# cmu-ci-lab/MitsubaER

Measured on AMD Instinct MI355X. Metric: Mpaths/sec (curved-ray heterogeneous volume); roofline = measured HBM GB/s of the dominant kernel vs peak, higher is better.
Workload: dtype f32; 1 GPU; configs[2]: 256^3 sigma_t grid + 256^3 linear-gradient RIF, RK4 eikonal curved rays, HG g=0.8, 512^2 x 256 spp; grid=256, spp_job=256, spp_per_gpu=256, pipelines_per_gpu=4, stepper=rk4, rif_interp=trilinear, layout=brick27, estimator=volpath + delta tracking on eikonal rays, ratio-tracking NEE, device=AMD Radeon Graphics, cus=256

## Files before the change

### mitsubaer_amd/csrc/mer_api.hip

```cpp
#include "mer_internal.hpp"
#define MER_USE_DEVICE(ctx) do { if (ctx) (void) hipSetDevice((ctx)->device); } while (0)
#include "mer_kernels.hpp"
#include <algorithm>
#include <functional>
#include <utility>

using namespace mer;

namespace { thread_local std::string g_create_error; }

namespace mer {

using FetchKinds = std::integer_sequence<int, RIFK_ACOUSTIC, MER_RIF_TRILINEAR, RIFK_DENSE_BUF, RIFK_CELL8, RIFK_CELL8_BUF, RIFK_BRICK27_BUF, RIFK_BRICK27, MER_RIF_BSPLINE3>;
using Steppers = std::integer_sequence<int, MER_STEP_VERLET, MER_STEP_RK4>;
template <int... Ks, typename F> static bool match_constant(std::integer_sequence<int, Ks...>, int value, F &&f) {
    return ((value == Ks && f(std::integral_constant<int, Ks>())) || ...);
}

template <typename F> static int dispatch_modes(mer_context *ctx, const mer_scene_desc *sc, F &&f) {
    const bool curved = sc->rif_mode != MER_RIF_CONST;
    const bool grid = sc->sigma_mode == MER_SIGMA_GRID;
    if (!curved) {
        if (grid) return f(std::integral_constant<bool, false>(), std::integral_constant<int, MER_RIF_TRILINEAR>(),
                           std::integral_constant<int, MER_STEP_VERLET>(), std::integral_constant<int, MER_SIGMA_GRID>(), std::integral_constant<int, 0>());
// ... 17 lines not shown

int mer_abi_version(void) { return MER_ABI_VERSION; }

int mer_context_create(int32_t device_id, mer_context **out) {
    if (!out) return 1;
    *out = nullptr;
    int ndev = 0;
    hipError_t e = hipGetDeviceCount(&ndev);
    if (e != hipSuccess || ndev <= 0) {
        g_create_error = "mer_context_create: no HIP device available (libmer has no CPU path)";
        return 1;
    }
    if (device_id < 0 || device_id >= ndev) { g_create_error = "mer_context_create: device id out of range"; return 1; }
    mer_context *ctx = new mer_context();
    ctx->device = device_id;
    if (hipSetDevice(device_id) != hipSuccess || hipGetDeviceProperties(&ctx->prop, device_id) != hipSuccess) {
        g_create_error = "mer_context_create: hipSetDevice failed"; delete ctx; return 1;
    }
    const size_t counter_bytes = sizeof(unsigned long long) * (MER_C_COUNT * MER_COUNTER_REPLICAS + 8);
    bool ok = !ctx->counters.alloc(ctx, counter_bytes) && hipMemset(ctx->counters.p, 0, counter_bytes) == hipSuccess &&
              hipEventCreate(&ctx->ev0) == hipSuccess && hipEventCreate(&ctx->ev1) == hipSuccess;
#ifdef MER_BOUNDS_CHECK
    ok = ok && !ctx->chk_buf.alloc(ctx, 4 * sizeof(unsigned long long)) && hipMemset(ctx->chk_buf.p, 0, 4 * sizeof(unsigned long long)) == hipSuccess;
    ctx->chk = ctx->chk_buf.as<unsigned long long>();
#endif
    if (!ok) { g_create_error = "mer_context_create: device allocation failed"; mer_context_destroy(ctx); return 1; }
    if (const char *e = getenv("MER_OPTIONS")) {
        std::string all(e); size_t pos = 0;
        while (pos < all.size()) {
            size_t end = all.find(',', pos); if (end == std::string::npos) end = all.size();
            const std::string kv = all.substr(pos, end - pos); const size_t eq = kv.find('=');
            if (eq != std::string::npos && mer_context_set_option(ctx, kv.substr(0, eq).c_str(), atoll(kv.c_str() + eq + 1)) != 0) {
                g_create_error = "mer_context_create: MER_OPTIONS: " + ctx->error; mer_context_destroy(ctx); return 1;
            }
            pos = end + 1;
        }
    }
    *out = ctx;
    return 0;
}

struct OptionEntry { const char *name; int64_t *p; int64_t min, max; };
static OptionEntry option_slot(mer_context *ctx, const char *name) {
    Options &o = ctx->opt;
    const int64_t ANY = INT64_MAX;
    const OptionEntry table[] = {
        {"pipes", &o.pipes, 1, MER_MAX_PIPES}, {"nslots", &o.nslots, 0, (int64_t) 1 << 28}, {"ksteps", &o.ksteps, 1, 1 << 20}, {"mq_sort", &o.mq_sort, -1, 1},
        {"connect_launches", &o.connect_launches, 1, 64}, {"adaptive_k", &o.adaptive_k, 0, 2}, {"pass_events", &o.pass_events, -ANY - 1, ANY},
        {"buffer_loads", &o.buffer_loads, -ANY - 1, ANY}, {"gen_all", &o.gen_all, -ANY - 1, ANY}, {"prefilter", &o.prefilter, 0, 5},
        {"verbose", &o.verbose, -ANY - 1, ANY}, {"debug_pixel", &o.debug_pixel, -1, ((int64_t) 1 << 31) - 1}, {"lds_bricks", &o.lds_bricks, -ANY - 1, ANY},
        {"march_lds_kb", &o.march_lds_kb, 0, 64},
        {"tile_deal", &o.tile_deal, 0, 1}, {"small_render_slots", &o.small_render_slots, 0, 1}, {"inline_walks", &o.inline_walks, 0, 1},
        {"spawn_walks", &o.spawn_walks, 0, 1}, {"grid_fit", &o.grid_fit, 0, 1}, {"check_every", &o.check_every, 1, 64},
        {"march_sort", &o.march_sort, 0, 4}, {"march_sort_major", &o.march_sort_major, 0, 1}};
    for (const auto &t : table) if (std::strcmp(t.name, name) == 0) return t;
    ctx->error = std::string("unknown option '") + name + "'";
    return OptionEntry{name, nullptr, 0, 0};
}
int mer_context_set_option(mer_context *ctx, const char *name, int64_t value) {
    MER_USE_DEVICE(ctx);
    if (!ctx || !name) return 1;
    const OptionEntry t = option_slot(ctx, name);
    if (!t.p) return 1;
    const bool nslots_too_few = t.p == &ctx->opt.nslots && value > 0 && value < MER_BLOCK * MER_MAX_PIPES;
    if (value < t.min || value > t.max || nslots_too_few) return fail(ctx, std::string("option '") + name + "': value out of range");
    *t.p = value;
    return 0;
}
int mer_context_get_option(mer_context *ctx, const char *name, int64_t *value) {
    MER_USE_DEVICE(ctx);
    if (!ctx || !name || !value) return 1;
    const OptionEntry t = option_slot(ctx, name);
    if (!t.p) return 1;
    *value = *t.p;
    return 0;
}
int mer_debug_bounds(mer_context *ctx, int32_t *enabled, uint64_t out[4]) {
    MER_USE_DEVICE(ctx);
    if (!ctx || !enabled || !out) return 1;
    out[0] = out[1] = out[2] = out[3] = 0;
    *enabled = ctx->chk != nullptr;
    if (ctx->chk) {
        HIP_CHECK(ctx, hipDeviceSynchronize());
        HIP_CHECK(ctx, hipMemcpy(out, ctx->chk, 4 * sizeof(uint64_t), hipMemcpyDeviceToHost));
        HIP_CHECK(ctx, hipMemset(ctx->chk, 0, 4 * sizeof(uint64_t)));
    }
    return 0;
}

void mer_context_destroy(mer_context *ctx) {
    if (!ctx) return;
    (void) hipSetDevice(ctx->device);
    for (Pipe &pp : ctx->pipes) {
        for (hipEvent_t e : pp.readback) if (e) (void) hipEventDestroy(e);
        if (pp.finished) (void) hipEventDestroy(pp.finished);
        for (hipEvent_t e : pp.pass_events) (void) hipEventDestroy(e);
        if (pp.own_stream) (void) hipStreamDestroy(pp.own_stream);
    }
    if (ctx->ev0) (void) hipEventDestroy(ctx->ev0);
    if (ctx->ev1) (void) hipEventDestroy(ctx->ev1);
    delete ctx;
}

const char *mer_last_error(mer_context *ctx) { return ctx ? ctx->error.c_str() : g_create_error.c_str(); }

int mer_context_set_stream(mer_context *ctx, void *hip_stream) { ctx->stream = (hipStream_t) hip_stream; return 0; }

// ... 719 lines not shown
```

### mitsubaer_amd/csrc/mer_device.hpp

```cpp
#pragma once
#include <hip/hip_runtime.h>
#include <stdint.h>
#include <stddef.h>
#include "../../include/mer.h"

#define MER_EPSILON 1e-4f
#define MER_PI 3.14159265358979323846f
#define MER_INV_FOURPI 0.07957747154594766788f
#define MER_INV_PI 0.31830988618379067154f
#define MER_INF __builtin_huge_valf()

namespace mer {

struct f3 {
    float x, y, z;
    __host__ __device__ __forceinline__ f3() {}
    __host__ __device__ __forceinline__ f3(float a, float b, float c) : x(a), y(b), z(c) {}
};
__device__ __forceinline__ f3 operator+(f3 a, f3 b) { return f3(a.x + b.x, a.y + b.y, a.z + b.z); }
__device__ __forceinline__ f3 operator-(f3 a, f3 b) { return f3(a.x - b.x, a.y - b.y, a.z - b.z); }
__device__ __forceinline__ f3 operator-(f3 a) { return f3(-a.x, -a.y, -a.z); }
__device__ __forceinline__ f3 operator*(f3 a, float s) { return f3(a.x * s, a.y * s, a.z * s); }
__device__ __forceinline__ f3 operator*(float s, f3 a) { return f3(s * a.x, s * a.y, s * a.z); }
__device__ __forceinline__ f3 operator*(f3 a, f3 b) { return f3(a.x * b.x, a.y * b.y, a.z * b.z); }
// ... 572 lines not shown
    float pad[2];
};
static_assert(sizeof(DPoint) == 32 && sizeof(DRect) == 160 && sizeof(DSpot) == 32 && sizeof(DEnvMap) == 144, "emitter records: 16-byte multiples");
struct EmitterTable { DPoint points[MER_MAX_EMITTERS]; DRect rects[MER_MAX_EMITTERS]; DSpot spots[MER_MAX_EMITTERS]; DEnvMap env; };
static_assert(offsetof(EmitterTable, spots) == offsetof(EmitterTable, rects) + sizeof(DRect) * MER_MAX_EMITTERS, "spot_table: the cones follow the rectangle table");
static_assert(offsetof(EmitterTable, env) == offsetof(EmitterTable, spots) + sizeof(DSpot) * MER_MAX_EMITTERS, "envmap_rec: the envmap record follows the cones");
static_assert(sizeof(EmitterTable) == offsetof(EmitterTable, env) + sizeof(DEnvMap), "emitter table: no padding (the host compares it bytewise)");

struct Params {
    mer_scene_desc sc;
    DGrid density, albedo, rif;
    f3    sigA, sigS, sigT;
    float medium_sampling_weight, sampling_density;
    MaxExp maxexp;
    float inv_max_density;
    float het_step;
    float aspect, cot_half_fov, par_dir[3], lens_radius, lens_focus, sensor_pad[1];
    float inv_res_x, inv_res_y;
    const float *ftable;
    float fradius, fscale;
    uint64_t seed;
    int32_t spp_begin, spp_count, spp_stride, tile_rank, tile_count;
    int32_t tiles_x, tiles_y, ntiles_mine;
    int32_t tile_skew;
    uint64_t total_work;
    float *film;
    int32_t frames, film_ch;
    float mod_phase;
    int32_t has_envmap;
    float *path_out;
    unsigned long long *counters;
    unsigned long long *work_counter;
    int32_t dbg_pixel;
    int32_t has_spot;
    uint32_t *slots; uint32_t nslots; int32_t ksteps;
    uint32_t nslots_all;
    int32_t spawn;
    uint32_t *live;
    SegQueue eq, mq[2], sq[2];
    DGrid sdf; float sdf_eps;
    SegQueue cq[2];
    uint32_t *cstate;
    unsigned long long *hitq; unsigned long long hitq_cap;
    unsigned long long *hitq_ctr;
    int32_t gen_iters, gen_all;
    uint32_t cq_row;
    int32_t mq_sort;
    int32_t msort, msort_major; float msort_o[3], msort_s[3];
    uint32_t *msorted, *msort_hist, *msort_cursor, *msort_count;
    unsigned long long *chk;
    uint64_t n_film, n_path_out;
    int32_t n_point, n_rect; const DPoint *points; const DRect *rects;
    uint8_t *side_state;
};
#define MER_LIVE_SLOTS 4096
#define MER_COUNTER_REPLICAS 64

__device__ __forceinline__ bool inside_shape(const mer_scene_desc &s, f3 p) {
    if (s.boundary == MER_BOUNDARY_SPHERE) {
        const f3 q(p.x - s.sph_center[0], p.y - s.sph_center[1], p.z - s.sph_center[2]);
        return dot(q, q) < s.sph_radius * s.sph_radius;
    }
    return p.x >= s.bmin[0] && p.x <= s.bmax[0] && p.y >= s.bmin[1] && p.y <= s.bmax[1] && p.z >= s.bmin[2] && p.z <= s.bmax[2];
}

__device__ __forceinline__ float intersect_shape(const mer_scene_desc &s, f3 o, f3 d, float mint, float maxt) {
    float nearT, farT;
    if (s.boundary == MER_BOUNDARY_SPHERE) {
        const double ox = (double) o.x - s.sph_center[0], oy = (double) o.y - s.sph_center[1], oz = (double) o.z - s.sph_center[2];
        const double dx = d.x, dy = d.y, dz = d.z;
        const double A = dx * dx + dy * dy + dz * dz, B = 2 * (dx * ox + dy * oy + dz * oz),
                     C = ox * ox + oy * oy + oz * oz - (double) s.sph_radius * s.sph_radius;
        const double disc = B * B - 4 * A * C;
        if (disc < 0) return -1.0f;
        const double root = sqrt(disc);
        const double q = B < 0 ? -0.5 * (B - root) : -0.5 * (B + root);
        double t0 = q / A, t1 = C / q;
        if (t0 > t1) { double tmp = t0; t0 = t1; t1 = tmp; }
        nearT = (float) t0; farT = (float) t1;
    } else {
        if (!aabb_intersect(s.bmin, s.bmax, o, d, nearT, farT)) return -1.0f;
    }
    if (!(nearT <= maxt && farT >= mint)) return -1.0f;
    if (nearT >= mint) return nearT;
    if (farT <= maxt) return farT;
    return -1.0f;
}

__device__ __forceinline__ void sample_ray(const Params &P, float px, float py, f3 &o, f3 &d, float &mint, float &maxt) {
    const float *cam = P.sc.cam_to_world;
    const float sx = px * P.inv_res_x, sy = py * P.inv_res_y;
    const f3 nearP((1.0f - 2.0f * sx) * P.sc.near_clip / P.cot_half_fov,
                   (1.0f - 2.0f * sy) / P.aspect * P.sc.near_clip / P.cot_half_fov, P.sc.near_clip);
    const f3 dl = normalize(nearP);
    const float invZ = 1.0f / dl.z;
    mint = P.sc.near_clip * invZ; maxt = P.sc.far_clip * invZ;
    o = f3(cam[3], cam[7], cam[11]);
    d = f3(cam[0] * dl.x + cam[1] * dl.y + cam[2] * dl.z,
           cam[4] * dl.x + cam[5] * dl.y + cam[6] * dl.z,
           cam[8] * dl.x + cam[9] * dl.y + cam[10] * dl.z);
}

__device__ __forceinline__ void square_to_disk_concentric(float u1, float u2, float &x, float &y) {
    const float r1 = 2.0f * u1 - 1.0f, r2 = 2.0f * u2 - 1.0f;
    float phi, r;
    if (r1 == 0 && r2 == 0) { r = phi = 0; }
// ... 513 lines not shown
```

### mitsubaer_amd/csrc/mer_internal.hpp

```cpp
#pragma once
#include "mer_device.hpp"
#include <cstdio>
#include <cstdlib>
#include <cstring>
#include <cmath>
#include <string>
#include <vector>
#include <map>
#include <limits>

struct mer_context;

namespace mer {

struct DeviceBuffer {
    void *p = nullptr; size_t bytes = 0;
    DeviceBuffer() = default;
    DeviceBuffer(DeviceBuffer &&o) noexcept : p(o.p), bytes(o.bytes) { o.p = nullptr; o.bytes = 0; }
    DeviceBuffer &operator=(DeviceBuffer &&o) noexcept { if (this != &o) { reset(); p = o.p; bytes = o.bytes; o.p = nullptr; o.bytes = 0; } return *this; }
    ~DeviceBuffer() { reset(); }
    void reset() { if (p) (void) hipFree(p); p = nullptr; bytes = 0; }
    void *release() { void *q = p; p = nullptr; bytes = 0; return q; }
    static int free_raw(mer_context *ctx, void *raw);
    int alloc(mer_context *ctx, size_t n);
// ... 33 lines not shown
    int32_t family = REC_FLUENCE, kind = REC_COLLISION;
    mer_fluence_desc box{};
    mer_detector_desc det{};
    int32_t frames = 0;
    DeviceBuffer dev;
    uint64_t n_keys = 0;
    int32_t n_totals = 0;
    bool timed() const { return kind == REC_TIMED; }
    bool track() const { return kind == REC_TRACK; }
    uint64_t n_cells() const { return (uint64_t) box.res[0] * (uint64_t) box.res[1] * (uint64_t) box.res[2]; }
    int32_t faces() const { return det.boundary == MER_BOUNDARY_SPHERE ? 1 : 6; }
    double *sums() const { return dev.as<double>(); }
    double *totals() const { return sums() + n_keys * 3; }
    size_t bytes() const { return (n_keys * 3 + (uint64_t) n_totals) * sizeof(double); }
};

#define MER_MAX_PIPES 4
struct Pipe {
    hipStream_t stream = nullptr, own_stream = nullptr;
    DeviceBuffer slots; uint32_t nslots = 0; DeviceBuffer live; PinnedBuffer host_live;
    enum { NQ = 7, EQ = 0, MQ = 1, SQ = 3, CQ = 5 };
    SegQueue q[NQ]{};
    DeviceBuffer q_items[NQ], q_counts[NQ], q_keys[NQ];
    DeviceBuffer cstate;
    DeviceBuffer hitq, hitq_ctr; unsigned long long hitq_cap = 0;
    hipEvent_t readback[2] = {nullptr, nullptr}, finished = nullptr;
    std::vector<hipEvent_t> pass_events;
    DeviceBuffer side_state;
    DeviceBuffer msort;
};

struct Options {
    int64_t pipes = 4;
    int64_t nslots = 0;
    int64_t ksteps = 128;
    int64_t mq_sort = -1;
    int64_t connect_launches = 2;
    int64_t adaptive_k = 0;
    int64_t pass_events = 1;
    int64_t buffer_loads = 1;
    int64_t gen_all = 0;
    int64_t prefilter = 0;
    int64_t verbose = 0;
    int64_t debug_pixel = -1;
    int64_t march_lds_kb = 0;
    int64_t tile_deal = 1;
    int64_t inline_walks = 1;
    int64_t spawn_walks = 1;
    int64_t small_render_slots = 1;
    int64_t check_every = 4;
    int64_t grid_fit = 1;
    int64_t march_sort = 0;
    int64_t march_sort_major = 0;
    int64_t lds_bricks = 0;
};

}

struct mer_context {
    int device = 0;
    hipStream_t stream = nullptr;
    std::string error;
    std::map<int, mer::Volume> volumes;
    std::map<int, mer::EnvMap> envmaps;
    std::map<int, mer::Recorder> recorders;
    mer::DeviceBuffer detect_list; uint32_t detect_cap = 0;
    int next_handle = 1;
    mer::DeviceBuffer counters;
    mer::DeviceBuffer ftable; int ftable_kind = -1; float ftable_param = 0;
    mer::DeviceBuffer etab; mer::EmitterTable etab_host; bool etab_valid = false;
    mer::DeviceBuffer chk_buf;
    unsigned long long *chk = nullptr;
    hipEvent_t ev0 = nullptr, ev1 = nullptr;
    bool timed = false;
    hipDeviceProp_t prop;
    mer::Options opt;
    mer::Pipe pipes[MER_MAX_PIPES];
    int last_passes = 0, last_pipes = 1;
    float last_march_ms = 0, last_event_ms = 0;
};

#define HIP_CHECK(ctx, call)                                                                              \
    do {                                                                                                  \
        hipError_t e_ = (call);                                                                           \
        if (e_ != hipSuccess) {                                                                           \
            (ctx)->error = std::string(#call) + " failed: " + hipGetErrorString(e_);                      \
            return 1;                                                                                     \
        }                                                                                                 \
    } while (0)

namespace mer {

inline int DeviceBuffer::free_raw(mer_context *ctx, void *raw) { HIP_CHECK(ctx, hipFree(raw)); return 0; }
inline int DeviceBuffer::alloc(mer_context *ctx, size_t n) {
    reset();
    HIP_CHECK(ctx, hipMalloc(&p, n ? n : 4));
    bytes = n;
    return 0;
}
inline int DeviceBuffer::upload(mer_context *ctx, const void *host, size_t n) {
    if (alloc(ctx, n)) return 1;
    if (n) HIP_CHECK(ctx, hipMemcpyAsync(p, host, n, hipMemcpyHostToDevice, ctx->stream));
    return 0;
}
inline int DeviceBuffer::download(mer_context *ctx, void *host, size_t n) const {
    if (n) HIP_CHECK(ctx, hipMemcpyAsync(host, p, n, hipMemcpyDeviceToHost, ctx->stream));
// ... 50 lines not shown
```

### mitsubaer_amd/csrc/mer_render.hip

```cpp
#include "mer_internal.hpp"
#include "mer_wavefront.hpp"
#include <chrono>

namespace mer {

static bool pick_kernels(mer_context *ctx, const mer_scene_desc *sc, bool extra, KernelSet &k) {
    const bool curved = sc->rif_mode != MER_RIF_CONST;
    const int sigma = sc->sigma_mode == MER_SIGMA_GRID ? MER_SIGMA_GRID : MER_SIGMA_HOMOGENEOUS;
    const int bnd = sc->boundary == MER_BOUNDARY_SDF ? 1 : 0;
    if (!curved) return kernels_straight(sigma, bnd, extra, k);
    const int rifk = rif_fetch_kind(ctx, sc);
    if (bnd) return kernels_sdf_curved(rifk, sc->stepper, sigma, k) || kernels_sdf_curved_records(rifk, sc->stepper, sigma, k);
    switch (rifk) {
    case RIFK_ACOUSTIC: return kernels_acoustic(sc->stepper, sigma, extra, k);
    case MER_RIF_TRILINEAR: case RIFK_DENSE_BUF: return kernels_dense(rifk, sc->stepper, sigma, extra, k);
    case RIFK_CELL8: case RIFK_CELL8_BUF: return kernels_cell8(rifk, sc->stepper, sigma, extra, k);
    case RIFK_BRICK27: case RIFK_BRICK27_BUF: return kernels_brick(rifk, sc->stepper, sigma, extra, k);
    case MER_RIF_BSPLINE3: return kernels_bspline(sc->stepper, sigma, extra, k);
    }
    return false;
}

int tile_skew_for(int tiles_x, int tile_count, int tile_deal) {
    if (tile_count <= 1 || tiles_x <= 1 || !tile_deal) return 0;
// ... 45 lines not shown
        __syncthreads();
        part[t] += v;
        __syncthreads();
    }
    const uint32_t excl = part[t] - sum;
#pragma unroll
    for (uint32_t k = 0; k < MER_SORT_MAXBINS / 1024; k++) { const uint32_t b = t * (MER_SORT_MAXBINS / 1024) + k; if (b < nb) { P.msort_cursor[b] = excl + loc[k]; P.msort_hist[b] = 0u; } }
    if (t == 1023) P.msort_count[0] = part[1023];
}
__global__ void __launch_bounds__(MER_BLOCK) msort_scatter_kernel(const Params P, uint32_t row) {
    __shared__ uint32_t h[MER_SORT_MAXBINS];
    const SegQueue q = pick_queue(P.mq, row);
    const uint32_t count = P.msort_count[0], base = blockIdx.x * MER_SORT_CHUNK, nb = msort_bins(P);
    if (base >= count) return;
    for (uint32_t b = threadIdx.x; b < nb; b += MER_BLOCK) h[b] = 0u;
    __syncthreads();
    uint32_t item[MER_SORT_CHUNK / MER_BLOCK], key[MER_SORT_CHUNK / MER_BLOCK], rank[MER_SORT_CHUNK / MER_BLOCK];
#pragma unroll
    for (uint32_t k = 0; k < MER_SORT_CHUNK / MER_BLOCK; k++) {
        const uint32_t j = base + k * MER_BLOCK + threadIdx.x;
        key[k] = 0xffffffffu;
        if (j < count) { uint32_t cls; const size_t at = msort_locate(q, row, j, cls); item[k] = q.items[at]; key[k] = msort_bin(P, q.keys[at], cls); rank[k] = atomicAdd(&h[key[k]], 1u); }
    }
    __syncthreads();
    for (uint32_t b = threadIdx.x; b < nb; b += MER_BLOCK) { const uint32_t c = h[b]; if (c) h[b] = atomicAdd(P.msort_cursor + b, c); }
    __syncthreads();
#pragma unroll
    for (uint32_t k = 0; k < MER_SORT_CHUNK / MER_BLOCK; k++)
        if (key[k] != 0xffffffffu) P.msorted[MER_CHK(P.chk, CHK_QUEUE_ITEM, h[key[k]] + rank[k], P.nslots_all)] = item[k];
}

int set_work(mer_context *ctx, const mer_scene_desc *scene, const mer_shard *shard, Params &P) {
    if (!shard || shard->spp_count < 0 || shard->spp_stride <= 0 || shard->tile_count <= 0 || shard->tile_rank < 0 ||
        shard->tile_rank >= shard->tile_count || shard->spp_begin < 0)
        return fail(ctx, "invalid shard");
    P.spp_begin = shard->spp_begin; P.spp_count = shard->spp_count; P.spp_stride = shard->spp_stride;
    P.tile_rank = shard->tile_rank; P.tile_count = shard->tile_count;
    P.tiles_x = (scene->width + MER_TILE - 1) / MER_TILE; P.tiles_y = (scene->height + MER_TILE - 1) / MER_TILE;
    P.tile_skew = tile_skew_for(P.tiles_x, shard->tile_count, (int) ctx->opt.tile_deal);
    const int ntiles = P.tiles_x * P.tiles_y;
    P.ntiles_mine = (ntiles - shard->tile_rank + shard->tile_count - 1) / shard->tile_count;
    P.total_work = (uint64_t) P.ntiles_mine * MER_TILE * MER_TILE * (uint64_t) shard->spp_count;
    return 0;
}

struct RenderPlan {
    KernelSet ks{};
    bool extra = false, connect_stage = false, spawn = false;
    uint32_t slot_mult = 1;
    int msort_bits = 0, npipes = 1, ksteps0 = 0, connect_launches = 0;
    uint32_t want = 0;
    unsigned gen_blocks_max = 1;
    unsigned long long ring = 1;
    uint64_t eq_segcap(uint32_t cap) const { return std::min<uint64_t>((uint64_t) cap, (uint64_t) ((connect_stage ? connect_launches : 0) + 2) * (cap / (MER_NSEG / MER_EV_CLASSES))) + 256u; }
    uint32_t segcap(int k, uint32_t cap) const {
        if (k == Pipe::EQ) return (uint32_t) eq_segcap(cap);
        if (k == Pipe::MQ || k == Pipe::MQ + 1) return 2u * (cap / (MER_NSEG / MER_MQ_CLASSES)) + 256u;
        if (k == Pipe::CQ || k == Pipe::CQ + 1) return cap + 256u;
        return 2u * (cap / MER_NSEG) + 256u;
    }
};

static int plan_render(mer_context *ctx, const mer_scene_desc *scene, const mer_shard *shard, const Params &P, bool point_outside, bool per_path, RenderPlan &pl) {
    const Options &opt = ctx->opt;
    const bool has_point = P.n_point > 0;
    const bool curved = scene->rif_mode != MER_RIF_CONST;
    const bool has_area = P.n_rect > 0;
    const bool extra = pl.extra = scene->boundary == MER_BOUNDARY_SDF || has_point || has_area || P.has_envmap || scene->modulation != MER_MODULATION_NONE || scene->boundary_bsdf != MER_BSDF_NULL
                       || scene->sensor != MER_SENSOR_PERSPECTIVE;
    KernelSet &ks = pl.ks;
    if (!pick_kernels(ctx, scene, extra, ks)) {
        if (scene->boundary == MER_BOUNDARY_SDF && curved) return fail(ctx, "signed-distance boundary: no kernel for this RIF layout (MER_LAYOUT_BRICK125 is not built with it)");
        return fail(ctx, "unsupported rif_mode / stepper combination");
    }
    if (opt.lds_bricks && ks.march_lds && curved) {
        auto it = ctx->volumes.find(scene->rif);
        if (it != ctx->volumes.end() && it->second.layout == MER_LAYOUT_BRICK27) ks.march = ks.march_lds;
    }
    const bool inline_walks = opt.inline_walks && ks.event_inline && !curved && scene->method != MER_METHOD_SIMPSON;
    if (inline_walks) ks.event = ks.event_inline;
    if (scene->boundary_bsdf == MER_BSDF_HROUGHDIELECTRIC) ks.event = inline_walks ? ks.event_inline_rough : ks.event_rough;
    const bool connect_stage = pl.connect_stage = has_point && curved && scene->boundary_bsdf != MER_BSDF_HROUGHDIELECTRIC;
    if (connect_stage && point_outside) ks.connect = ks.connect_cross;

    const bool has_env = scene->env_radiance[0] != 0 || scene->env_radiance[1] != 0 || scene->env_radiance[2] != 0;
    const bool spawn = pl.spawn = opt.spawn_walks && curved && !extra && has_env && !per_path && scene->decomposition == MER_DECOMPOSITION_NONE;
    pl.slot_mult = spawn ? 1u + 2u * MER_SIDE_PER_KIND : 1u;
    pl.msort_bits = (curved && !extra && scene->boundary != MER_BOUNDARY_SDF && P.rif.res[0] > 1 && P.rif.wmax[0] > P.rif.wmin[0]) ? (int) opt.march_sort : 0;
    int npipes = (int) opt.pipes;
    if (shard->spp_count < npipes) npipes = std::max(1, shard->spp_count);
    uint32_t want = opt.nslots > 0 ? (uint32_t) opt.nslots : (uint32_t) ctx->prop.multiProcessorCount * 2048u * 4u;
    if (opt.nslots == 0 && opt.small_render_slots && P.total_work / 8 < want) want = (uint32_t) std::max<uint64_t>(want / 4, P.total_work / 8);
    pl.want = want = (want / (uint32_t) npipes + MER_BLOCK - 1) / MER_BLOCK * MER_BLOCK;
    pl.npipes = npipes; pl.ksteps0 = (int) opt.ksteps;
    pl.connect_launches = (int) opt.connect_launches;
    const unsigned gen_blocks_max = pl.gen_blocks_max = std::max(1u, std::min(want / MER_BLOCK, 1024u));
    const unsigned long long ids_per_launch = (unsigned long long) gen_blocks_max * (MER_BLOCK / 64) * 64ull * (unsigned long long) P.gen_iters;
    unsigned long long ring = 1; while (ring < 2ull * std::max<unsigned long long>(want, ids_per_launch)) ring <<= 1;
    pl.ring = ring;
    return 0;
}

static int prepare_pool(mer_context *ctx, const RenderPlan &pl, const Params &P, const mer_shard *shard, int q, Run &R) {
    Pipe &pp = ctx->pipes[q];
    const uint32_t want = pl.want, slot_mult = pl.slot_mult;
    if (q == 0) pp.stream = ctx->stream;
    else if (!pp.own_stream) { HIP_CHECK(ctx, hipStreamCreateWithFlags(&pp.own_stream, hipStreamNonBlocking)); }
    if (q > 0) { pp.stream = pp.own_stream; HIP_CHECK(ctx, hipStreamWaitEvent(pp.stream, ctx->ev0, 0)); }
    if (pp.nslots < want * slot_mult || pp.hitq_cap < pl.ring || (pp.nslots && pp.q[Pipe::EQ].segcap < pl.eq_segcap(pp.nslots))) {
        const uint32_t cap = std::max(want * slot_mult, pp.nslots);
        pp.nslots = 0;
        if (pp.slots.reserve(ctx, (size_t) cap * MER_SLOT_WORDS * sizeof(uint32_t))) return 1;
        for (int k = 0; k < Pipe::NQ; k++) {
            SegQueue &sq = pp.q[k];
            sq.segcap = pl.segcap(k, cap);
            if (pp.q_items[k].reserve(ctx, (size_t) sq.segcap * MER_NSEG * sizeof(uint32_t)) ||
                pp.q_counts[k].reserve(ctx, (size_t) MER_LIVE_SLOTS * MER_NSEG * sizeof(uint32_t))) return 1;
            sq.items = pp.q_items[k].as<uint32_t>(); sq.counts = pp.q_counts[k].as<uint32_t>(); sq.chk = ctx->chk;
        }
        pp.hitq_cap = std::max(pl.ring, pp.hitq_cap);
        if (pp.hitq.reserve(ctx, (size_t) pp.hitq_cap * sizeof(unsigned long long))) return 1;
        pp.nslots = cap;
    }
    if (pp.live.reserve(ctx, MER_LIVE_SLOTS * sizeof(uint32_t)) || (!pp.host_live.p && pp.host_live.alloc(ctx, 8 * sizeof(uint32_t))) ||
        pp.hitq_ctr.reserve(ctx, 64 * sizeof(unsigned long long))) return 1;
    for (hipEvent_t *e : {&pp.readback[0], &pp.readback[1], &pp.finished}) if (!*e) HIP_CHECK(ctx, hipEventCreateWithFlags(e, hipEventDisableTiming));
    R.P = P;
    R.P.spp_begin = shard->spp_begin + q * shard->spp_stride; R.P.spp_stride = shard->spp_stride * pl.npipes;
    R.P.spp_count = (shard->spp_count - q + pl.npipes - 1) / pl.npipes;
    R.P.total_work = (uint64_t) P.ntiles_mine * MER_TILE * MER_TILE * (uint64_t) R.P.spp_count;
    R.nslots = want;
    const uint64_t need_slots = (R.P.total_work + MER_BLOCK - 1) / MER_BLOCK * MER_BLOCK;
    if (need_slots < R.nslots) R.nslots = (uint32_t) need_slots;
    uint32_t *slots = pp.slots.as<uint32_t>();
    R.P.slots = slots; R.P.nslots = R.nslots; R.P.nslots_all = R.nslots * slot_mult; R.P.spawn = pl.spawn ? 1 : 0; R.P.live = pp.live.as<uint32_t>();
    R.P.eq = pp.q[Pipe::EQ];
    for (int k = 0; k < 2; k++) { R.P.mq[k] = pp.q[Pipe::MQ + k]; R.P.sq[k] = pp.q[Pipe::SQ + k]; R.P.cq[k] = pp.q[Pipe::CQ + k]; }
    if (pl.connect_stage && pp.cstate.reserve(ctx, (size_t) pp.nslots * MER_CSTATE_WORDS * sizeof(uint32_t))) return 1;
    R.P.cstate = pp.cstate.as<uint32_t>();
    if (pl.spawn && pp.side_state.reserve(ctx, (size_t) want * 8u)) return 1;
    R.P.side_state = pl.spawn ? pp.side_state.as<uint8_t>() : nullptr;
    R.P.msort = 0; R.P.mq[0].keys = nullptr; R.P.mq[1].keys = nullptr;
    if (pl.msort_bits) {
        if (pp.msort.reserve(ctx, ((size_t) pp.nslots + 2 * MER_SORT_MAXBINS + 16) * sizeof(uint32_t))) return 1;
        for (int k = 0; k < 2; k++) {
            DeviceBuffer &keys = pp.q_keys[Pipe::MQ + k];
            if (keys.reserve(ctx, (size_t) R.P.mq[k].segcap * MER_NSEG * sizeof(uint16_t))) return 1;
            R.P.mq[k].keys = keys.as<uint16_t>();
        }
        R.P.msort = std::min(pl.msort_bits, P.mq_sort ? 3 : 4); R.P.msort_major = (int) ctx->opt.march_sort_major;
        R.P.msorted = pp.msort.as<uint32_t>();
        R.P.msort_hist = R.P.msorted + pp.nslots; R.P.msort_cursor = R.P.msort_hist + MER_SORT_MAXBINS; R.P.msort_count = R.P.msort_cursor + MER_SORT_MAXBINS;
        for (int k = 0; k < 3; k++) { R.P.msort_o[k] = P.rif.wmin[k]; const float e = P.rif.wmax[k] - P.rif.wmin[k]; R.P.msort_s[k] = e > 0 ? (float) (1 << R.P.msort) / e : 0.0f; }
        HIP_CHECK(ctx, hipMemsetAsync(R.P.msort_hist, 0, (2 * MER_SORT_MAXBINS + 16) * sizeof(uint32_t), pp.stream));
    }
    R.P.hitq = pp.hitq.as<unsigned long long>(); R.P.hitq_cap = pp.hitq_cap; R.P.hitq_ctr = pp.hitq_ctr.as<unsigned long long>(); R.P.work_counter = R.P.hitq_ctr + 48;
    R.P.ksteps = pl.ksteps0; R.P.cq_row = 0;
    R.done = R.P.total_work == 0;
    if (R.done) return 0;
    R.blocks = R.nslots * slot_mult / MER_BLOCK;
    R.alive_bound = R.nslots; R.child_bound = R.nslots * (slot_mult - 1u);
    R.gen_blocks = std::max(1u, std::min(R.nslots / MER_BLOCK, pl.gen_blocks_max));
    HIP_CHECK(ctx, hipMemsetAsync(slots, 0, (size_t) R.nslots * MER_SLOT_WORDS * sizeof(uint32_t), pp.stream));
    if (pl.spawn) hipLaunchKernelGGL(clear_side_flags_kernel, dim3(nblocks((int64_t) R.nslots * (slot_mult - 1u))), dim3(256), 0, pp.stream, slots, R.nslots, R.nslots * slot_mult);
    if (pl.spawn) HIP_CHECK(ctx, hipMemsetAsync(pp.side_state.p, 0, (size_t) R.nslots * 8u, pp.stream));
    HIP_CHECK(ctx, hipMemsetAsync(pp.live.p, 0, MER_LIVE_SLOTS * sizeof(uint32_t), pp.stream));
    for (DeviceBuffer &counts : pp.q_counts)
        HIP_CHECK(ctx, hipMemsetAsync(counts.p, 0, (size_t) MER_LIVE_SLOTS * MER_NSEG * sizeof(uint32_t), pp.stream));
    HIP_CHECK(ctx, hipMemsetAsync(pp.hitq_ctr.p, 0, 64 * sizeof(unsigned long long), pp.stream));
    return 0;
}

int launch_render(mer_context *ctx, const mer_scene_desc *scene, const mer_shard *shard, uint64_t seed, float *film_dev, float *path_out_dev,
                  uint64_t n_film, uint64_t n_path_out) {
    Params P; bool point_outside = false;
    if (make_params(ctx, scene, P, true, &point_outside)) return 1;
    if (set_work(ctx, scene, shard, P)) return 1;
    const Options &opt = ctx->opt;
    P.seed = seed;
    P.film = film_dev; P.path_out = path_out_dev; P.n_film = n_film; P.n_path_out = n_path_out;
    HIP_CHECK(ctx, hipSetDevice(ctx->device));
    if (P.total_work == 0) return 0;
    P.mq_sort = opt.mq_sort >= 0 ? (opt.mq_sort != 0) : ((int64_t) P.rif.res[0] * P.rif.res[1] * P.rif.res[2] <= ((int64_t) 1 << 28) ? 1 : 0);
    P.gen_iters = 8; P.gen_all = opt.gen_all ? 1 : 0;
    RenderPlan pl;
    if (plan_render(ctx, scene, shard, P, point_outside, path_out_dev != nullptr, pl)) return 1;
    const KernelSet &ks = pl.ks; const bool connect_stage = pl.connect_stage; const uint32_t slot_mult = pl.slot_mult;
    const int npipes = pl.npipes, ksteps0 = pl.ksteps0, connect_launches = pl.connect_launches;

    Run runs[MER_MAX_PIPES];
    const auto t_start = std::chrono::steady_clock::now();
    HIP_CHECK(ctx, hipEventRecord(ctx->ev0, ctx->stream));
    for (int q = 0; q < npipes; q++) if (prepare_pool(ctx, pl, P, shard, q, runs[q])) return 1;

    const uint32_t check_every = (uint32_t) opt.check_every;
    const bool pass_events = opt.pass_events != 0;
    const bool side_walks_return = scene->sigma_mode == MER_SIGMA_GRID && scene->tr_estimator == MER_TR_WOODCOCK2;
    auto enqueue_batch = [&](int q, int rb) -> int {
        Pipe &pp = ctx->pipes[q]; Run &R = runs[q];
        uint32_t *host_live = (uint32_t *) pp.host_live.p;
        unsigned march_blocks = R.blocks, event_blocks = R.blocks;
        if (opt.grid_fit) {
            const uint64_t records = std::min<uint64_t>((uint64_t) R.nslots * slot_mult, (uint64_t) R.alive_bound * slot_mult + R.child_bound);
            march_blocks = (unsigned) std::max<uint64_t>(1, (records + MER_BLOCK - 1) / MER_BLOCK);
            event_blocks = side_walks_return ? march_blocks : (unsigned) std::max<uint64_t>(1, ((uint64_t) R.alive_bound + MER_BLOCK - 1) / MER_BLOCK);
        }
        for (uint32_t b = 0; b < check_every; b++) {
            const uint32_t pass = R.pass;
            while (pp.pass_events.size() < (size_t) (pass + 1) * 3) {
                hipEvent_t e; HIP_CHECK(ctx, hipEventCreate(&e)); pp.pass_events.push_back(e);
            }
            if (pass_events) HIP_CHECK(ctx, hipEventRecord(pp.pass_events[pass * 3 + 0], pp.stream));
            for (int g = 0; R.work_left && g < (pass == 0 ? 6 : 1); g++) hipLaunchKernelGGL(ks.gen, dim3(R.gen_blocks), dim3(MER_BLOCK), 0, pp.stream, R.P);
            hipLaunchKernelGGL(ks.event, dim3(event_blocks), dim3(MER_BLOCK), 0, pp.stream, R.P, pass);
            for (int l = 0; connect_stage && l < connect_launches; l++) {
                hipLaunchKernelGGL(ks.connect, dim3(event_blocks), dim3(MER_BLOCK), 0, pp.stream, R.P, pass);
                R.P.cq_row++;
            }
            if (pass_events) HIP_CHECK(ctx, hipEventRecord(pp.pass_events[pass * 3 + 1], pp.stream));
            if (R.P.msort) {
                const unsigned sb = (unsigned) (((uint64_t) march_blocks * MER_BLOCK + MER_SORT_CHUNK - 1) / MER_SORT_CHUNK);
                hipLaunchKernelGGL(msort_hist_kernel, dim3(sb), dim3(MER_BLOCK), 0, pp.stream, R.P, pass);
                hipLaunchKernelGGL(msort_scan_kernel, dim3(1), dim3(1024), 0, pp.stream, R.P);
                hipLaunchKernelGGL(msort_scatter_kernel, dim3(sb), dim3(MER_BLOCK), 0, pp.stream, R.P, pass);
            }
            hipLaunchKernelGGL(ks.march, dim3(march_blocks), dim3(MER_BLOCK), (size_t) opt.march_lds_kb * 1024, pp.stream, R.P, pass);
            if (pass_events) HIP_CHECK(ctx, hipEventRecord(pp.pass_events[pass * 3 + 2], pp.stream));
            R.pass++;
        }
        HIP_CHECK(ctx, hipGetLastError());
        HIP_CHECK(ctx, hipMemcpyAsync(host_live + 4 * rb, pp.live.p, 2 * sizeof(uint32_t), hipMemcpyDeviceToHost, pp.stream));
        HIP_CHECK(ctx, hipMemcpyAsync(host_live + 4 * rb + 2, R.P.work_counter, sizeof(unsigned long long), hipMemcpyDeviceToHost, pp.stream));
        HIP_CHECK(ctx, hipEventRecord(pp.readback[rb], pp.stream));
        return 0;
    };
    auto abort_render = [&]() -> int {
        const std::string msg = ctx->error;
        for (int q = 0; q < npipes; q++) if (ctx->pipes[q].stream || q == 0) (void) hipStreamSynchronize(q == 0 ? ctx->stream : ctx->pipes[q].stream);
        ctx->error = msg;
        return 1;
    };
    for (int q = 0; q < npipes; q++) if (!runs[q].done && enqueue_batch(q, 0)) return abort_render();
    for (int q = 0; q < npipes; q++) if (!runs[q].done && enqueue_batch(q, 1)) return abort_render();
    for (;;) {
        bool any = false;
        for (int q = 0; q < npipes; q++) {
            Pipe &pp = ctx->pipes[q]; Run &R = runs[q];
            const uint32_t *host_live = (uint32_t *) pp.host_live.p;
            if (R.done) continue;
            any = true;
            const int rb = R.cur; R.cur ^= 1;
            if (hipEventSynchronize(pp.readback[rb]) != hipSuccess) { ctx->error = "hipEventSynchronize(readback) failed"; return abort_render(); }
            const uint32_t finished_slots = host_live[4 * rb];
            if (opt.verbose >= 2)
                fprintf(stderr, "[mer] t=%8.3f ms pipe %d passes %u finished %u / %u work %llu / %llu K=%d\n", std::chrono::duration<double, std::milli>(std::chrono::steady_clock::now() - t_start).count(),
                        q, R.pass, finished_slots, R.nslots, *(unsigned long long *) (host_live + 4 * rb + 2), (unsigned long long) R.P.total_work, R.P.ksteps);
            if (finished_slots >= R.nslots && host_live[4 * rb + 1] == 0u) { R.done = true; continue; }
            R.alive_bound = R.nslots - std::min(finished_slots, R.nslots); R.child_bound = host_live[4 * rb + 1];
            R.work_left = *(unsigned long long *) (host_live + 4 * rb + 2) < R.P.total_work;
// ... 39 lines not shown
```

### mitsubaer_amd/csrc/mer_wavefront.hpp

```cpp
#pragma once
#include "mer_walk.hpp"
#include "mer_connect.hpp"
#include "mer_microfacet.hpp"

namespace mer {

enum { H_PX = 0, H_PY, H_PZ, H_VX, H_VY, H_VZ, H_OPT, H_DIST, H_REM, H_HPREV, H_TR, H_T, H_TMAX, H_STEPS, H_FLAGS,
       H_RNG_LO, H_RNG_HI, H_PIXEL, H_SAMPLE, H_SIGMA, H_COUNT };
enum { CO_PXF = H_COUNT, CO_PYF, CO_LX, CO_LY, CO_LZ, CO_TX, CO_TY, CO_TZ, CO_DEPTH, CO_PFLAGS, CO_PSX, CO_PSY, CO_PSZ,
       CO_DSX, CO_DSY, CO_DSZ, CO_DDX, CO_DDY, CO_DDZ, CO_WIX, CO_WIY, CO_WIZ, CO_PHASEPDF, CO_ITST, CO_N0, CO_TRSUM,
       CO_SDENS, CO_TMIN, CO_WNEXT_LO, CO_WNEXT_HI, CO_WLEFT, CO_PLEN, CO_TROPT, CO_ETA, SLOT_WORDS };

#define MER_FLAG_INIT (1u << 13)
#define MER_FLAG_CHILD (1u << 14)
__device__ __forceinline__ uint32_t pack_flags(int st, int ev, int kind, int seg_inf, int backstep, int walk, int agg) {
    return (uint32_t) st | ((uint32_t) ev << 2) | ((uint32_t) kind << 6) | ((uint32_t) seg_inf << 8) | ((uint32_t) backstep << 9) |
           ((uint32_t) walk << 10) | ((uint32_t) agg << 12);
}

#define MER_SLOT_WORDS 64
#define MER_HITQ_HEAD 32
#ifndef MER_WORK_BATCH
#define MER_WORK_BATCH 8
#endif
#define SLOT(k) P.slots[(size_t) MER_CHK(P.chk, CHK_SLOT, i, P.nslots_all) * MER_SLOT_WORDS + (k)]
#define SLOTF(k) __uint_as_float(SLOT(k))

template <class WalkT>
__device__ __forceinline__ void load_hot(const Params &P, uint32_t i, uint32_t &fl, WalkT &W, Rng &rng, uint32_t &pixel, uint32_t &sample, float &sigma) {
    const uint4 *r = (const uint4 *) (P.slots + (size_t) MER_CHK(P.chk, CHK_SLOT, i, P.nslots_all) * MER_SLOT_WORDS);
    const uint4 a = r[0], b = r[1], c = r[2], d = r[3], e = r[4];
    W.p = f3(__uint_as_float(a.x), __uint_as_float(a.y), __uint_as_float(a.z));
    W.v = f3(__uint_as_float(a.w), __uint_as_float(b.x), __uint_as_float(b.y));
    W.opt = __uint_as_float(b.z); W.dist = __uint_as_float(b.w);
    W.rem = __uint_as_float(c.x); W.hprev = __uint_as_float(c.y); W.Tr = __uint_as_float(c.z); W.t = __uint_as_float(c.w);
    W.tmax = __uint_as_float(d.x); W.steps_left = (int) d.y; fl = d.z;
    rng.state = (uint64_t) d.w | ((uint64_t) e.x << 32);
    pixel = e.y; sample = e.z; sigma = __uint_as_float(e.w);
    W.kind = (fl >> 6) & 3; W.seg_inf = (fl >> 8) & 1; W.backstep = (fl >> 9) & 1; W.walk = (fl >> 10) & 3;
    W.agg = (fl >> 12) & 1; W.dleft = sigma;
    rng.inc = (((((uint64_t) sample) << 32) | (uint64_t) pixel) << 1) | 1ULL;
}
template <class WalkT>
__device__ __forceinline__ void store_hot(const Params &P, uint32_t i, int st, int ev, const WalkT &W, const Rng &rng,
                                          uint32_t pixel, uint32_t sample, float sigma, uint32_t keep_bits = 0u) {
    uint4 *r = (uint4 *) (P.slots + (size_t) MER_CHK(P.chk, CHK_SLOT, i, P.nslots_all) * MER_SLOT_WORDS);
    r[0] = make_uint4(__float_as_uint(W.p.x), __float_as_uint(W.p.y), __float_as_uint(W.p.z), __float_as_uint(W.v.x));
    r[1] = make_uint4(__float_as_uint(W.v.y), __float_as_uint(W.v.z), __float_as_uint(W.opt), __float_as_uint(W.dist));
    r[2] = make_uint4(__float_as_uint(W.rem), __float_as_uint(W.hprev), __float_as_uint(W.Tr), __float_as_uint(W.t));
    const bool agg = WalkT::kBND == 1 && W.agg != 0;
    r[3] = make_uint4(__float_as_uint(W.tmax), (uint32_t) W.steps_left, pack_flags(st, ev, W.kind, W.seg_inf, W.backstep, W.walk, agg ? 1 : 0) | keep_bits,
                      (uint32_t) rng.state);
    r[4] = make_uint4((uint32_t) (rng.state >> 32), pixel, sample, __float_as_uint((WalkT::kBND == 1 && ev == EV_NONE) ? W.dleft : sigma));
}

#define MER_COLD_WORDS 36
// ... 254 lines not shown
        float dist;
        if (S.boundary == MER_BOUNDARY_SPHERE) {
            const f3 q(W.p.x - S.sph_center[0], W.p.y - S.sph_center[1], W.p.z - S.sph_center[2]);
            const float b = dot(q, W.v) * __builtin_amdgcn_rsqf(vv), c0 = dot(q, q) - S.sph_radius * S.sph_radius;
            dist = sqrtf(fmaxf(b * b - c0, 0.0f)) - b;
        } else {
            const float tx = ((W.v.x > 0 ? S.bmax[0] : S.bmin[0]) - W.p.x) * __builtin_amdgcn_rcpf(W.v.x),
                        ty = ((W.v.y > 0 ? S.bmax[1] : S.bmin[1]) - W.p.y) * __builtin_amdgcn_rcpf(W.v.y),
                        tz = ((W.v.z > 0 ? S.bmax[2] : S.bmin[2]) - W.p.z) * __builtin_amdgcn_rcpf(W.v.z);
            dist = fminf(fminf(tx, ty), tz) * sqrtf(vv);
        }
        r = dist * __builtin_amdgcn_rcpf(S.stepsize);
    } else r = (W.tmax - W.t) * __builtin_amdgcn_rcpf(P.inv_max_density);
    const float f = CURVED ? r * ((float) (MER_MQ_CLASSES - 1) * __builtin_amdgcn_rcpf((float) P.ksteps)) : 0.5f * r;
    return f >= (float) (MER_MQ_CLASSES - 1) ? 0 : (MER_MQ_CLASSES - 1) - (int) fmaxf(f, 0.0f);
}
__device__ __forceinline__ uint32_t queue_total(const SegQueue &q, uint32_t row) {
    const uint32_t *c = q.counts + (size_t) (row & (MER_LIVE_SLOTS - 1)) * MER_NSEG;
    uint32_t t = 0;
#pragma unroll
    for (int s = 0; s < MER_NSEG; s++) t += c[s];
    return t;
}
__device__ __forceinline__ uint32_t queue_item(const SegQueue &q, uint32_t row, uint32_t j) {
    const uint32_t *c = q.counts + (size_t) (row & (MER_LIVE_SLOTS - 1)) * MER_NSEG;
    uint32_t seg = 0, off = j;
#pragma unroll
    for (int s = 0; s < MER_NSEG - 1; s++) { const uint32_t n = c[s]; if (seg == (uint32_t) s && off >= n) { off -= n; seg = s + 1; } }
    return q.items[(size_t) seg * q.segcap + MER_CHK(q.chk, CHK_QUEUE_ITEM, off, q.segcap)];
}
__device__ __forceinline__ void queue_clear_row(const SegQueue &q, uint32_t row, uint32_t j) {
    if (j < MER_NSEG) q.counts[(size_t) (row & (MER_LIVE_SLOTS - 1)) * MER_NSEG + j] = 0;
}

#define MER_SORT_CHUNK 2048u
#define MER_SORT_MAXBINS 4096u
__device__ __forceinline__ uint32_t msort_bin(const Params &P, uint32_t cell, uint32_t cls) {
    if (!P.mq_sort) return cell;
    return P.msort_major ? (cls << (3 * P.msort)) + cell : cell * MER_MQ_CLASSES + cls;
}
__device__ __forceinline__ uint32_t msort_bins(const Params &P) { return (P.mq_sort ? (uint32_t) MER_MQ_CLASSES : 1u) << (3 * P.msort); }

#ifndef MER_MARCH_WAVES
#define MER_MARCH_WAVES 4
#endif
#ifndef MER_ARRIVE_BATCH
#define MER_ARRIVE_BATCH 4
#endif
template <bool CURVED, int RIF, int STEPPER, int SIGMA, int BND = 0>
__global__ void __launch_bounds__(MER_BLOCK, MER_MARCH_WAVES) march_kernel(const Params P, uint32_t pass) {
    const uint32_t j = blockIdx.x * MER_BLOCK + threadIdx.x;
    if (j >= P.nslots_all) return;
    if (j == 0) { const unsigned long long t = P.hitq_ctr[0], h = P.hitq_ctr[MER_HITQ_HEAD]; if (h > t) P.hitq_ctr[MER_HITQ_HEAD] = t; }
    const uint32_t count = P.msort ? P.msort_count[0] : queue_total(P.mq[pass & 1u], pass);
    uint32_t jl = j;
    if (P.msort) {
        const uint32_t T = (count + MER_BLOCK - 1) / MER_BLOCK, b = blockIdx.x, x = b & 7u, qd = T >> 3, r = T & 7u;
        jl = b < T ? ((x < r ? x * (qd + 1u) : r * (qd + 1u) + (x - r) * qd) + (b >> 3)) * MER_BLOCK + threadIdx.x : 0xffffffffu;
    }
    LaneCounters C; C.clear();
    uint32_t iters = 0, i = 0;
    bool has_event = false, still_marching = false, child_ended = false; int ev_class = 0, mq_class = 0;
    if (jl < count) {
        i = P.msort ? P.msorted[jl] : queue_item(P.mq[pass & 1u], pass, jl);
        uint32_t fl;
        Walk<CURVED, RIF, STEPPER, SIGMA, BND> W;
        Rng rng; uint32_t pixel, sample; float sigma;
        load_hot(P, i, fl, W, rng, pixel, sample, sigma);
        W.cc.reset(); W.n0 = 1.0f; W.tmin = 0.0f; W.trsum = 0.0f; W.sdens = 0.0f;
        int ev = EV_NONE; sigma = 0.0f;
        if (CURVED && (fl & MER_FLAG_INIT)) {
            ev = W.begin(P, rng, C, W.kind, W.p, W.v, W.t);
            if (!(fl & MER_FLAG_CHILD)) { W.tmax = W.n0; if (SIGMA != MER_SIGMA_GRID) SLOT(CO_SDENS) = __float_as_uint(W.sdens); }
        }
        const int K = ev == EV_NONE ? P.ksteps : 0;
        if (CURVED) {
            bool pend = false; uint32_t nadv = 0;
            for (int k = 0; k < K; ++k) {
                if (!pend) {
                    ev = W.template advance<false>(P, rng, C); nadv++;
                    if (ev == EV_ARRIVED) { pend = true; ev = EV_NONE; }
                }
                if (((k & (MER_ARRIVE_BATCH - 1)) == MER_ARRIVE_BATCH - 1 || k == K - 1) && pend) { ev = W.on_arrived(P, rng, C, sigma); pend = false; }
                iters++;
                if (ev != EV_NONE) break;
            }
            C.marched += nadv; C.steps += nadv; C.rif_evals += nadv * evals_per_step<STEPPER>();
        } else
        for (int k = 0; k < K; ++k) {
            ev = W.advance(P, rng, C);
            if (ev == EV_ARRIVED) ev = W.on_arrived(P, rng, C, sigma);
            iters++;
            if (ev != EV_NONE) break;
        }
        const bool child = CURVED && BND == 0 && (fl & MER_FLAG_CHILD) != 0u;
        if (child && ev != EV_NONE && !(SIGMA == MER_SIGMA_GRID && P.sc.tr_estimator == MER_TR_WOODCOCK2)) {
            f3 tr = SIGMA == MER_SIGMA_GRID ? f3(W.Tr, W.Tr, W.Tr) : homogeneous_transmittance(P, -W.dist);
            if (ev == EV_GATE_FAIL) tr = f3(0, 0, 0);
            const uint4 q = *(const uint4 *) (P.slots + (size_t) MER_CHK(P.chk, CHK_SLOT, i, P.nslots_all) * MER_SLOT_WORDS + CO_PXF);
            const f3 c = f3(__uint_as_float(q.z), __uint_as_float(q.w), SLOTF(CO_LZ)) * tr;
            if (!is_zero(c)) film_splat(P, __uint_as_float(q.x), __uint_as_float(q.y), c, 0.0f, 0, 1);
            SLOT(H_FLAGS) = 0u; side_state_clear(P, __float_as_uint(W.tmax));
            child_ended = true; ev = EV_NONE;
        } else
        store_hot(P, i, ST_MARCH, ev, W, rng, pixel, sample, sigma, fl & MER_FLAG_CHILD);
        has_event = ev != EV_NONE;
        ev_class = ev == EV_REAL ? 0 : (W.kind == K_NEE ? 1 : (W.kind == K_LOOKUP ? 2 : 3));
        mq_class = march_class<CURVED, BND>(P, W);
        still_marching = !has_event && !child_ended;
    }
    queue_push_class<MER_EV_CLASSES>(P.eq, pass + 1, has_event, i, ev_class);
    queue_push_class<MER_MQ_CLASSES>(P.mq[(pass + 1) & 1u], pass + 1, still_marching, i, mq_class & 255, (uint32_t) mq_class >> 8);
// ... 621 lines not shown
```

Before: 369.6 Mpaths/s.

## Spread sparse march queue items across more wavefronts to raise occupancy

When the march queue holds fewer items than a budget of wavefronts, items are redistributed so each wave handles only a few lanes' worth of work, and the march launch is enlarged to at least the spread budget (default 5120 waves split across pipelines). The aim is to stop tail passes with few live paths from packing into a handful of full waves on a few CUs, and to spread long RK4 marches across many CUs. The cost is more launched blocks, partially filled wavefronts, and lower SIMD utilisation per wave.

```diff
diff --git a/mitsubaer_amd/csrc/mer_api.hip b/mitsubaer_amd/csrc/mer_api.hip
--- a/mitsubaer_amd/csrc/mer_api.hip
+++ b/mitsubaer_amd/csrc/mer_api.hip
@@ -93,7 +93,8 @@
         {"march_lds_kb", &o.march_lds_kb, 0, 64},
         {"tile_deal", &o.tile_deal, 0, 1}, {"small_render_slots", &o.small_render_slots, 0, 1}, {"inline_walks", &o.inline_walks, 0, 1},
         {"spawn_walks", &o.spawn_walks, 0, 1}, {"grid_fit", &o.grid_fit, 0, 1}, {"check_every", &o.check_every, 1, 64},
-        {"march_sort", &o.march_sort, 0, 4}, {"march_sort_major", &o.march_sort_major, 0, 1}};
+        {"march_sort", &o.march_sort, 0, 4}, {"march_sort_major", &o.march_sort_major, 0, 1},
+        {"march_spread", &o.march_spread, 0, 1 << 20}};
     for (const auto &t : table) if (std::strcmp(t.name, name) == 0) return t;
     ctx->error = std::string("unknown option '") + name + "'";
     return OptionEntry{name, nullptr, 0, 0};
diff --git a/mitsubaer_amd/csrc/mer_device.hpp b/mitsubaer_amd/csrc/mer_device.hpp
--- a/mitsubaer_amd/csrc/mer_device.hpp
+++ b/mitsubaer_amd/csrc/mer_device.hpp
@@ -648,6 +648,7 @@
     uint64_t n_film, n_path_out;
     int32_t n_point, n_rect; const DPoint *points; const DRect *rects;
     uint8_t *side_state;
+    uint32_t march_spread;
 };
 #define MER_LIVE_SLOTS 4096
 #define MER_COUNTER_REPLICAS 64
diff --git a/mitsubaer_amd/csrc/mer_internal.hpp b/mitsubaer_amd/csrc/mer_internal.hpp
--- a/mitsubaer_amd/csrc/mer_internal.hpp
+++ b/mitsubaer_amd/csrc/mer_internal.hpp
@@ -109,6 +109,7 @@
     int64_t grid_fit = 1;
     int64_t march_sort = 0;
     int64_t march_sort_major = 0;
+    int64_t march_spread = 5120;
     int64_t lds_bricks = 0;
 };
 
diff --git a/mitsubaer_amd/csrc/mer_march_spread.hpp b/mitsubaer_amd/csrc/mer_march_spread.hpp
--- /dev/null
+++ b/mitsubaer_amd/csrc/mer_march_spread.hpp
@@ -0,0 +1,23 @@
+#pragma once
+#include <stdint.h>
+#if defined(__HIPCC__) || defined(__CUDACC__)
+#define MER_SPREAD_HD __host__ __device__ __forceinline__
+#else
+#define MER_SPREAD_HD inline
+#endif
+
+namespace mer {
+
+#define MER_SPREAD_NONE 0xffffffffu
+
+MER_SPREAD_HD uint32_t march_spread_pos(uint32_t wave, uint32_t lane, uint32_t count, uint32_t grid_waves, uint32_t budget) {
+    const uint32_t waves = grid_waves < budget ? grid_waves : budget;
+    uint32_t pos = wave * 64u + lane;
+    if (waves != 0u && (count >> 6) < waves) {
+        const uint32_t L = (count + waves - 1u) / waves;
+        pos = (wave < waves && lane < L) ? wave * L + lane : MER_SPREAD_NONE;
+    }
+    return pos < count ? pos : MER_SPREAD_NONE;
+}
+
+}
diff --git a/mitsubaer_amd/csrc/mer_render.hip b/mitsubaer_amd/csrc/mer_render.hip
--- a/mitsubaer_amd/csrc/mer_render.hip
+++ b/mitsubaer_amd/csrc/mer_render.hip
@@ -121,6 +121,7 @@
     uint32_t want = 0;
     unsigned gen_blocks_max = 1;
     unsigned long long ring = 1;
+    uint32_t march_spread = 0;
     uint64_t eq_segcap(uint32_t cap) const { return std::min<uint64_t>((uint64_t) cap, (uint64_t) ((connect_stage ? connect_launches : 0) + 2) * (cap / (MER_NSEG / MER_EV_CLASSES))) + 256u; }
     uint32_t segcap(int k, uint32_t cap) const {
         if (k == Pipe::EQ) return (uint32_t) eq_segcap(cap);
@@ -162,6 +163,7 @@
     if (opt.nslots == 0 && opt.small_render_slots && P.total_work / 8 < want) want = (uint32_t) std::max<uint64_t>(want / 4, P.total_work / 8);
     pl.want = want = (want / (uint32_t) npipes + MER_BLOCK - 1) / MER_BLOCK * MER_BLOCK;
     pl.npipes = npipes; pl.ksteps0 = (int) opt.ksteps;
+    pl.march_spread = (uint32_t) (opt.march_spread / npipes);
     pl.connect_launches = (int) opt.connect_launches;
     const unsigned gen_blocks_max = pl.gen_blocks_max = std::max(1u, std::min(want / MER_BLOCK, 1024u));
     const unsigned long long ids_per_launch = (unsigned long long) gen_blocks_max * (MER_BLOCK / 64) * 64ull * (unsigned long long) P.gen_iters;
@@ -224,7 +226,7 @@
         HIP_CHECK(ctx, hipMemsetAsync(R.P.msort_hist, 0, (2 * MER_SORT_MAXBINS + 16) * sizeof(uint32_t), pp.stream));
     }
     R.P.hitq = pp.hitq.as<unsigned long long>(); R.P.hitq_cap = pp.hitq_cap; R.P.hitq_ctr = pp.hitq_ctr.as<unsigned long long>(); R.P.work_counter = R.P.hitq_ctr + 48;
-    R.P.ksteps = pl.ksteps0; R.P.cq_row = 0;
+    R.P.ksteps = pl.ksteps0; R.P.cq_row = 0; R.P.march_spread = R.P.msort ? 0u : pl.march_spread;
     R.done = R.P.total_work == 0;
     if (R.done) return 0;
     R.blocks = R.nslots * slot_mult / MER_BLOCK;
@@ -274,6 +276,7 @@
             march_blocks = (unsigned) std::max<uint64_t>(1, (records + MER_BLOCK - 1) / MER_BLOCK);
             event_blocks = side_walks_return ? march_blocks : (unsigned) std::max<uint64_t>(1, ((uint64_t) R.alive_bound + MER_BLOCK - 1) / MER_BLOCK);
         }
+        march_blocks = std::max(march_blocks, std::min(R.blocks, (unsigned) (R.P.march_spread / (MER_BLOCK / 64))));
         for (uint32_t b = 0; b < check_every; b++) {
             const uint32_t pass = R.pass;
             while (pp.pass_events.size() < (size_t) (pass + 1) * 3) {
diff --git a/mitsubaer_amd/csrc/mer_wavefront.hpp b/mitsubaer_amd/csrc/mer_wavefront.hpp
--- a/mitsubaer_amd/csrc/mer_wavefront.hpp
+++ b/mitsubaer_amd/csrc/mer_wavefront.hpp
@@ -2,6 +2,7 @@
 #include "mer_walk.hpp"
 #include "mer_connect.hpp"
 #include "mer_microfacet.hpp"
+#include "mer_march_spread.hpp"
 
 namespace mer {
 
@@ -362,12 +363,14 @@
     const uint32_t j = blockIdx.x * MER_BLOCK + threadIdx.x;
     if (j >= P.nslots_all) return;
     if (j == 0) { const unsigned long long t = P.hitq_ctr[0], h = P.hitq_ctr[MER_HITQ_HEAD]; if (h > t) P.hitq_ctr[MER_HITQ_HEAD] = t; }
+    const uint32_t spread_waves = min(gridDim.x * (MER_BLOCK / 64), P.march_spread);
     const uint32_t count = P.msort ? P.msort_count[0] : queue_total(P.mq[pass & 1u], pass);
     uint32_t jl = j;
     if (P.msort) {
         const uint32_t T = (count + MER_BLOCK - 1) / MER_BLOCK, b = blockIdx.x, x = b & 7u, qd = T >> 3, r = T & 7u;
         jl = b < T ? ((x < r ? x * (qd + 1u) : r * (qd + 1u) + (x - r) * qd) + (b >> 3)) * MER_BLOCK + threadIdx.x : 0xffffffffu;
-    }
+    } else if ((count >> 6) < spread_waves)
+        jl = march_spread_pos(j >> 6, threadIdx.x & 63u, count, spread_waves, spread_waves);
     LaneCounters C; C.clear();
     uint32_t iters = 0, i = 0;
     bool has_event = false, still_marching = false, child_ended = false; int ev_class = 0, mq_class = 0;
```

After: 371.6 Mpaths/s, median of 6. No clear change (+0.5%).
